# cbrl/BNN-PYNQ

Measured on AMD Instinct MI355X. Metric: images/sec (whole node) CNV-W1A1 CIFAR-10-shape batch, higher is better.
Workload: dtype u1; 1 GPU; cnvW1A1, 131072 synthetic 32x32x3 uint8 images per GPU per step, inputs resident in HBM, params cifar10/cnvW1A1; parallelism=dp1 (batch shards, no data-path collective)

## Files before the change

bnn-pynq_amd/bnn/abi.py:

```python
import ctypes as C
import os

ROOT = os.path.dirname(os.path.realpath(__file__))
PLATFORM = os.environ.get("BNN_PLATFORM", "mi355x")
LIB_DIR = os.environ.get("BNN_MI355X_LIBDIR") or os.path.join(ROOT, "libraries", PLATFORM)
PARAM_ROOT = os.path.join(ROOT, "params")

LEGACY = ["load_parameters", "inference", "inference_multiple", "inference_multiple_with_faults",
          "free_results", "deinit"]
EXT = ["bnn_mi355x_network", "bnn_mi355x_image_bytes", "bnn_mi355x_last_error", "bnn_mi355x_set_device",
       "bnn_mi355x_pack_params", "bnn_mi355x_export_params", "bnn_mi355x_import_params",
       "bnn_mi355x_inference_buffer", "bnn_mi355x_inference_raw", "bnn_mi355x_inference_device",
       "bnn_mi355x_reserve", "bnn_mi355x_set_fault_seed", "bnn_mi355x_last_faults", "bnn_mi355x_plan_faults",
       "bnn_mi355x_pack_params_faulty", "bnn_mi355x_debug_stage_output", "bnn_mi355x_profile",
       "bnn_mi355x_profile_read", "bnn_mi355x_stage_name", "bnn_mi355x_thumbnail_size", "bnn_mi355x_images_to_cifar",
       "bnn_mi355x_params_bytes", "bnn_mi355x_import_params_device", "bnn_mi355x_params_crc", "bnn_mi355x_chunk_plan",
       "bnn_mi355x_binarize_pack", "bnn_mi355x_fault_campaigns", "bnn_mi355x_last_campaign_faults",
       "bnn_mi355x_enumerate_faults", "bnn_mi355x_fault_sweep", "bnn_mi355x_last_sweep_stages",
       "bnn_mi355x_enumerate_act_faults", "bnn_mi355x_act_fault_sweep", "bnn_mi355x_last_act_sweep_stages",
       "bnn_mi355x_matrix_stages", "bnn_mi355x_act_noise_campaigns", "bnn_mi355x_last_act_noise_counts",
       "bnn_mi355x_last_act_noise_seeds", "bnn_mi355x_act_noise_mask", "bnn_mi355x_enumerate_input_faults",
       "bnn_mi355x_input_fault_sweep", "bnn_mi355x_last_input_sweep_stages", "bnn_mi355x_input_noise_campaigns",
       "bnn_mi355x_last_input_noise_counts", "bnn_mi355x_last_input_noise_seeds", "bnn_mi355x_input_noise_mask",
       "bnn_mi355x_sweep_profile", "bnn_mi355x_last_sweep_profile", "bnn_mi355x_mem_noise_campaigns",
       "bnn_mi355x_last_mem_noise_counts", "bnn_mi355x_last_mem_noise_seeds", "bnn_mi355x_mem_noise_mask",
       "bnn_mi355x_mem_noise_params", "bnn_mi355x_hardening_scheme", "bnn_mi355x_hardening_layout", "bnn_mi355x_hardened_site",
       "bnn_mi355x_hardened_mem_noise_mask", "bnn_mi355x_pack_params_hardened", "bnn_mi355x_hardened_mem_noise_campaigns",
       "bnn_mi355x_hardened_mem_noise_params", "bnn_mi355x_last_hardened_mem_noise_counts",
       "bnn_mi355x_last_hardened_mem_noise_seeds", "bnn_mi355x_exposure_mask", "bnn_mi355x_exposure_campaigns",
       "bnn_mi355x_exposure_params", "bnn_mi355x_last_exposure_counts", "bnn_mi355x_last_exposure_seeds", "bnn_mi355x_ecc_encode",
       "bnn_mi355x_ecc_decode", "bnn_mi355x_ecc_layout", "bnn_mi355x_ecc_check_site", "bnn_mi355x_ecc_exposure_mask",
       "bnn_mi355x_pack_params_ecc", "bnn_mi355x_ecc_exposure_campaigns", "bnn_mi355x_ecc_exposure_params",
       "bnn_mi355x_last_ecc_exposure_counts", "bnn_mi355x_last_ecc_exposure_seeds", "bnn_mi355x_ecc_repair",
       "bnn_mi355x_pack_params_repair", "bnn_mi355x_repair_exposure_campaigns", "bnn_mi355x_repair_exposure_params",
       "bnn_mi355x_last_repair_exposure_counts", "bnn_mi355x_last_repair_exposure_seeds", "bnn_mi355x_wecc_encode",
       "bnn_mi355x_wecc_decode", "bnn_mi355x_wecc_repair", "bnn_mi355x_wecc_layout", "bnn_mi355x_wecc_exposure_mask",
       "bnn_mi355x_pack_params_wecc", "bnn_mi355x_wecc_exposure_campaigns", "bnn_mi355x_wecc_exposure_params",
       "bnn_mi355x_last_wecc_exposure_counts", "bnn_mi355x_last_wecc_exposure_seeds", "bnn_mi355x_iwecc_layout",
       "bnn_mi355x_iwecc_site", "bnn_mi355x_pack_params_iwecc", "bnn_mi355x_iwecc_exposure_campaigns",
       "bnn_mi355x_iwecc_exposure_params", "bnn_mi355x_last_iwecc_exposure_counts", "bnn_mi355x_last_iwecc_exposure_seeds",
       "bnn_mi355x_tile_boxes", "bnn_mi355x_windows_to_cifar", "bnn_mi355x_classify_windows"]


def lib_path(network, runtime="python_sw", lib_dir=None):
    return os.path.join(lib_dir or LIB_DIR, "%s-%s-%s.so" % (runtime, network, PLATFORM))


def declare_legacy(L):
    ip, fp = C.POINTER(C.c_int), C.POINTER(C.c_float)
    L.load_parameters.argtypes = [C.c_char_p]
    L.load_parameters.restype = None
    L.inference.argtypes = [C.c_char_p, ip, C.c_int, fp]
    L.inference.restype = C.c_int
    L.inference_multiple.argtypes = [C.c_char_p, C.c_int, ip, fp, C.c_int]
    L.inference_multiple.restype = ip
    L.inference_multiple_with_faults.argtypes = [C.c_char_p, C.c_int, ip, fp, C.c_uint, C.c_int, C.c_int, ip, C.c_uint]
    L.inference_multiple_with_faults.restype = ip
    L.free_results.argtypes = [ip]
    L.free_results.restype = None
    L.deinit.argtypes = []
    L.deinit.restype = None


def declare_extensions(L):
# ... 212 lines not shown
```

bnn-pynq_amd/csrc/kernels.h:

```cpp
#pragma once
#include <hip/hip_runtime.h>
#include <stdint.h>

#include "topology.h"

namespace bnn {

struct CnvLaunch {
  const uint8_t *images;
  int n;
  void *buf0, *buf1;
  const uint32_t *rows[9];
  const uint8_t *l0_mfma;
  const uint8_t *l1_mfma;
  const uint8_t *conv_mfma;
  bool l1_literal;
  bool has_two;
  int16_t *scores;
  int32_t *classes;
  int number_class;
  hipStream_t stream;
  hipEvent_t *events;
  int last_stage;
  hipEvent_t t0, t1;
  unsigned *done_flag;
  unsigned done_seq;
};

struct LfcLaunch {
  const uint8_t *images;
  bool packed;
  int n;
  void *buf0, *buf1;
  const uint32_t *rows[4];
  uint64_t *words;
  int32_t *classes;
  int number_class;
  hipStream_t stream;
  hipEvent_t *events;
  int last_stage;
  hipEvent_t t0, t1;
  bool t_dispatch;
  unsigned *done_flag;
  unsigned done_seq;
};

constexpr int kL0TileOffset = 2 * 64 * 32, kL0BigBytes = 2 * 32 * 2 * 16;

constexpr int kCnvStages = 9;
constexpr int kLfcStages = 6;
const char *stage_name(bool is_cnv, int stage);

size_t stage_output_bytes(bool is_cnv, int abits, int stage, int *in_buf1);
void cnv_workspace_bytes(int abits, size_t *buf0, size_t *buf1);
void lfc_workspace_bytes(int abits, size_t *buf0, size_t *buf1);

constexpr size_t kL1MfmaWeights = 9 * 2 * 64 * 16, kL1MfmaBytes = kL1MfmaWeights + 2 * 2 * 16 * 4;
void l1_mfma_table(const uint32_t *rows, uint8_t *dst);

constexpr size_t kConvMfmaL2Off = kL1MfmaBytes, kConvMfmaL3Off = kConvMfmaL2Off + 9 * 4 * 64 * 16 + 4 * 32 * 4,
                 kTailMfmaL4Off = kConvMfmaL3Off + 18 * 4 * 64 * 16 + 4 * 32 * 4;
constexpr size_t kTailMfmaL5Off = kTailMfmaL4Off + 18 * 8 * 64 * 16 + 8 * 32 * 4, kTailMfmaL6Off = kTailMfmaL5Off + 36 * 8 * 64 * 16 + 8 * 32 * 4,
                 kTailMfmaL7Off = kTailMfmaL6Off + 4 * 16 * 64 * 16 + 16 * 32 * 4, kConvMfmaBytes = kTailMfmaL7Off + 8 * 16 * 64 * 16 + 16 * 32 * 4;
hipError_t conv_mfma_table(const uint32_t *const rows[9], uint8_t *dst, hipStream_t s);

constexpr size_t kConvMfmaA2L2Off = 9 * 2 * 64 * 16 + 2 * 64 * 4, kConvMfmaA2L3Off = kConvMfmaA2L2Off + 9 * 4 * 64 * 16 + 4 * 64 * 4,
                 kTailMfmaA2L4Off = kConvMfmaA2L3Off + 18 * 4 * 64 * 16 + 4 * 64 * 4;
constexpr size_t kTailMfmaA2L5Off = kTailMfmaA2L4Off + 18 * 8 * 64 * 16 + 8 * 64 * 4, kTailMfmaA2L6Off = kTailMfmaA2L5Off + 36 * 8 * 64 * 16 + 8 * 64 * 4,
                 kTailMfmaA2L7Off = kTailMfmaA2L6Off + 4 * 16 * 64 * 16 + 16 * 64 * 4, kConvMfmaA2Bytes = kTailMfmaA2L7Off + 8 * 16 * 64 * 16 + 16 * 64 * 4;
hipError_t conv_mfma_a2_table(NetId net, const uint32_t *const rows[9], uint8_t *dst, hipStream_t s);

int cnv_matrix_stages(NetId net, const CnvLaunch &a);

hipError_t run_cnv(NetId net, const CnvLaunch &a);
hipError_t run_lfc(NetId net, const LfcLaunch &a);

struct MultiSeg { int run, image, slot, len; };
struct MultiLaunch {
  const uint8_t *images;
  const MultiSeg *segs;
  int nsegs, max_len, total;
  int n;
  void *buf0, *buf1;
  const uint32_t *rows[9];
  const uint8_t *l0_mfma;
  size_t stride;
  bool has_two;
  int32_t *classes;
  uint64_t *words;
  int number_class;
  hipStream_t stream;
  int first = 0, last = 1 << 30;
};
hipError_t run_cnv_multi(NetId net, const MultiLaunch &a);
hipError_t run_lfc_multi(NetId net, const MultiLaunch &a);
// ... 65 lines not shown
```

bnn-pynq_amd/csrc/kernels.hip:

```cpp
#include <hip/hip_runtime.h>
#include <hip/hip_ext.h>
#include <stdint.h>

#include <cstdlib>
#include <cstring>
#include <type_traits>

#define BNN_HD __host__ __device__
#include "act_faults.h"
#include "input_faults.h"
#include "kernels.h"
#include "mem_faults.h"
#include "mem_org.h"
#include "packed_params.h"
static_assert(bnn::kL0TileOffset == (int)bnn::kL0MfmaTileOffset && bnn::kL0BigBytes == (int)bnn::kL0MfmaBigBytes,
              "k_conv0_tile's operand offsets must be the ones packed_params.cpp writes the layer-0 table by");

namespace bnn {
namespace {

typedef const uint32_t __attribute__((address_space(4))) *kptr32;
typedef const uint64_t __attribute__((address_space(4))) *kptr64;

constexpr int kBlock = 256;
// ... 595 lines not shown
        if (valid && h == 0 && !(c & 1)) gout[(size_t)(t0 >> 1) * NT + (c >> 1) * NT + mt] = ~pooled;
      } else {
        uint32_t nf[2];
#pragma unroll
        for (int dy = 0; dy < 2; dy++) {
          int v[16];
#pragma unroll
          for (int k = 0; k < 16; k++) v[k] = __float_as_int(acc[dy][k]);
          nf[dy] = sign_nibbles(v, h);
        }
        const auto sw = __builtin_amdgcn_permlane32_swap(nf[0], nf[1], false, false);
        if (valid) *reinterpret_cast<uint32_t *>(reinterpret_cast<char *>(gout) + ob) = ~(sw[0] | sw[1]);
      }
      x += DX, rp += DR, ps += 2 * DR * WS + DX;
      if constexpr (!POOL) ob += (2 * DR * WOUT + DX) * NT * 4;
      if (x >= WOUT) {
        x -= WOUT, rp += 1, ps += 2 * WS - WOUT;
        if constexpr (!POOL) ob += WOUT * NT * 4;
      }
      if (rp >= RP) rp -= RP, ps += IMGS - 2 * RP * WS;
    }
  }
}

__global__ __launch_bounds__(256) void k_conv_mfma_table(const uint32_t *__restrict__ rows, int row_dw, int ksteps, int tiles,
                                                          int mw, uint8_t *__restrict__ dst) {
  const int idx = blockIdx.x * 256 + threadIdx.x, nw = ksteps * tiles * 64;
  if (idx < nw) {
    const int ks = idx / (tiles * 64), mt = (idx / 64) % tiles, lane = idx & 63, n = 32 * mt + (lane & 31), h = lane >> 5;
    const uint32_t bits = rows[(size_t)n * row_dw + 2 + 2 * ks + h];
    reinterpret_cast<uint4 *>(dst)[idx] = make_uint4(fp4_pm1(bits & 255), fp4_pm1((bits >> 8) & 255), fp4_pm1((bits >> 16) & 255),
                                                     fp4_pm1(bits >> 24));
  } else if (idx < nw + tiles * 32) {
    const int j = idx - nw, mt = j >> 5, h = (j >> 4) & 1, reg = j & 15;
    const int n = 32 * mt + (reg & 3) + 8 * (reg >> 2) + 4 * h;
    long long t = (int)rows[(size_t)n * row_dw];
    t = t < -1 ? -1 : (t > mw + 2 ? mw + 2 : t);
    reinterpret_cast<float *>(dst + (size_t)nw * 16)[j] = (float)(-(mw - 2 * t) - 1);
  }
}

__device__ __forceinline__ uint32_t nibble_spread(uint32_t byte) {
  uint32_t t = byte & 0xFFu;
  t = (t | (t << 12)) & 0x000F000Fu;
  t = (t | (t << 6)) & 0x03030303u;
  return (t | (t << 3)) & 0x11111111u;
// ... 2044 lines not shown
  else return a.n >= conv_mfma_a2_min<ARITH>() ? a.conv_mfma : nullptr;
}
constexpr long long kTailMfmaMinW1A1 = 3072, kTailMfmaMinW1A2 = 3072, kTailMfmaMinW2A2 = 1024;
constexpr int kTailMfmaStages = 0xF0;
template <int ARITH>
inline long long tail_mfma_min() {
  static const long long v = [] {
    const char *e = std::getenv("BNN_MI355X_TAIL_MFMA_MIN");
    return e ? std::atoll(e) : (ARITH == AR_XNOR ? kTailMfmaMinW1A1 : ARITH == AR_TB ? kTailMfmaMinW1A2 : kTailMfmaMinW2A2);
  }();
  return v;
}
template <int ARITH>
inline const uint8_t *tail_mfma_for(const CnvLaunch &a) {
  if (a.done_flag && a.n == 1) return nullptr;
  return a.n >= tail_mfma_min<ARITH>() ? a.conv_mfma : nullptr;
}
inline unsigned persistent_grid(long long units, long long cap) {
  const long long per = (units + cap - 1) / cap;
  return (unsigned)((units + per - 1) / per);
}
constexpr long long kConvMfmaGrid = 512;
constexpr int kConvMfmaImgsL1 = 2, kConvMfmaImgs = 8;
constexpr int kTailMfmaImgsL4 = 32, kTailMfmaImgsL5 = 32, kTailMfmaImgsFc = 128;
constexpr long long kTailMfmaGrid8 = 256;
#define BNN_TAIL_MFMA(A2, KS, NT, CONV, WAVES, G, cap, in, out, tab)                                                               \
  hipLaunchKernelGGL((k_tail_mfma<A2, KS, NT, CONV, WAVES, G>), dim3(persistent_grid((n + (G) - 1) / (G), (cap))), dim3(64 * (WAVES)), 0, s, \
                     in, out, tab, (int)n)

inline int gpb_for(long long items, int groups) { return (items + kBlock - 1) / kBlock >= 2048 ? groups : 1; }

inline bool narrow_for(long long items, int groups32, long long limit) { return ((items + kBlock - 1) / kBlock) * groups32 < limit; }
constexpr long long kNarrowLimitCnv = 8192, kNarrowLimitLfc = 512;
constexpr long long kFcLastWaveMax = 32768;
constexpr long long kPixelLaneMax = 512;
constexpr long long kCnvTailMax = 1024;

inline dim3 grid_for(long long items, int groups) {
  const long long item_blocks = (items + kBlock - 1) / kBlock;
  return dim3((unsigned)(((item_blocks + 7) / 8) * 8 * groups));
}

#define BNN_LAUNCH(kern, grid, stream, ...)                                   \
  do {                                                                        \
    if ((grid).x > 0) hipLaunchKernelGGL(kern, grid, dim3(kBlock), 0, stream, __VA_ARGS__); \
  } while (0)
// ... 18 lines not shown
  if (a.l0_mfma) {
    const dim3 g0((unsigned)((n * 900 + kBlock - 1) / kBlock));
    if (a.last_stage >= 0) {
      if (n >= l0_tile_min()) BNN_LAUNCH((k_conv0_tile<OUT2>), dim3((unsigned)((n + kL0Imgs - 1) / kL0Imgs)), s, a.images, A, a.l0_mfma, (int)n);
      else BNN_LAUNCH((k_conv0_mfma<OUT2>), g0, s, a.images, A, a.l0_mfma, (int)(n * 900));
    }
  } else {
    if (a.last_stage >= 0) BNN_LAUNCH((k_conv0<OUT2>), grid_for(n * 900, 2 / gpb_for(n * 900, 2)), s, a.images, A, a.rows[0], (int)(n * 900), 2, gpb_for(n * 900, 2));
  }
  BNN_MARK(a.events, 1, s);
  if constexpr (ARITH == AR_XNOR && !OUT2) {
    const bool pix = n <= kPixelLaneMax;
    const uint8_t *const cm = conv_mfma_for<ARITH, OUT2>(a);
    const dim3 g1(persistent_grid((n + kConvMfmaImgsL1 - 1) / kConvMfmaImgsL1, kConvMfmaGrid)),
        gm(persistent_grid((n + kConvMfmaImgs - 1) / kConvMfmaImgs, kConvMfmaGrid));
    if (a.last_stage >= 1) {
      if (a.l1_literal) {
        BNN_LAUNCH(k_l1_literal, dim3((unsigned)((n * 784 + kBlock - 1) / kBlock)), s, A64, reinterpret_cast<uint64_t *>(B), a.rows[1], (int)(n * 784));
      } else if (a.l1_mfma) {
        const long long pairs = (n + 1) / 2;
        hipLaunchKernelGGL(k_l1_mfma, dim3((unsigned)(pairs < 512 ? pairs : 512)), dim3(256), 0, s, reinterpret_cast<const uint32_t *>(a.buf0), B,
                           a.l1_mfma, (int)n);
      } else if (cm) {
        hipLaunchKernelGGL((k_conv_mfma<30, 2, 2, true, kConvMfmaImgsL1>), g1, dim3(256), 0, s, reinterpret_cast<const uint32_t *>(a.buf0), B, cm,
                           (int)n);
      } else if (pix) BNN_LAUNCH((k_vec_x<9, true, 1, 30, 8, true>), grid_for(n * 784, 8), s, A64, B, a.rows[1], (int)(n * 784), 8, 1);
      else BNN_STAGE((k_quad_x<1, 30, true>), (k_quad_x<1, 30, true, 8>), n * 196, 2, A64, B, a.rows[1]);
    }
    BNN_MARK(a.events, 2, s);
    if (a.last_stage >= 2) {
      if (cm) hipLaunchKernelGGL((k_conv_mfma<14, 2, 4, false, kConvMfmaImgs>), gm, dim3(256), 0, s, B, A, cm + kConvMfmaL2Off, (int)n);
      else if (pix) BNN_LAUNCH((k_vec_x<9, true, 1, 14, 8>), grid_for(n * 144, 16), s, B64, A, a.rows[2], (int)(n * 144), 16, 1);
      else BNN_STAGE((k_quad_x<1, 14, false>), (k_quad_x<1, 14, false, 8>), n * 36, 4, B64, A, a.rows[2]);
    }
    BNN_MARK(a.events, 3, s);
    if (a.last_stage >= 3) {
      if (cm) hipLaunchKernelGGL((k_conv_mfma<12, 4, 4, true, kConvMfmaImgs>), gm, dim3(256), 0, s, A, B, cm + kConvMfmaL3Off, (int)n);
      else if (pix) BNN_LAUNCH((k_vec_x<18, true, 2, 12, 8, true>), grid_for(n * 100, 16), s, A64, B, a.rows[3], (int)(n * 100), 16, 1);
      else BNN_STAGE((k_quad_x<2, 12, true>), (k_quad_x<2, 12, true, 8>), n * 25, 4, A64, B, a.rows[3]);
    }
    BNN_MARK(a.events, 4, s);
    const uint8_t *const tm = tail_mfma_for<ARITH>(a);
    const uint32_t *const A32 = A, *const B32 = B;
    if (!tm && n <= kCnvTailMax && !a.events && a.last_stage >= kCnvStages - 1) {
      hipLaunchKernelGGL(k_cnv_tail, dim3((unsigned)n), dim3(512), 0, s, B64, a.scores, a.classes, a.rows[4], a.rows[5], a.rows[6],
                         a.rows[7], a.rows[8], a.number_class, n == 1 ? a.done_flag : nullptr, a.done_seq);
      return;
    }
    if (a.last_stage >= 4) {
      if (tm && (kTailMfmaStages & 16)) BNN_TAIL_MFMA(false, 18, 8, true, 8, kTailMfmaImgsL4, kTailMfmaGrid8, B32, A, tm + kTailMfmaL4Off);
      else BNN_STAGE((k_vec_x<18, true, 2, 5>), (k_vec_x<18, true, 2, 5, 8>), n * 9, 8, B64, A, a.rows[4]);
    }
    BNN_MARK(a.events, 5, s);
    if (a.last_stage >= 5) {
      if (tm && (kTailMfmaStages & 32)) BNN_TAIL_MFMA(false, 36, 8, false, 8, kTailMfmaImgsL5, kTailMfmaGrid8, A32, B, tm + kTailMfmaL5Off);
      else BNN_STAGE((k_vec_x<36, false, 1, 1>), (k_vec_x<36, false, 1, 1, 8>), n, 8, A64, B, a.rows[5]);
    }
    BNN_MARK(a.events, 6, s);
    if (a.last_stage >= 6) {
      if (tm && (kTailMfmaStages & 64)) BNN_TAIL_MFMA(false, 4, 16, false, 4, kTailMfmaImgsFc, kConvMfmaGrid, B32, A, tm + kTailMfmaL6Off);
// ... 208 lines not shown
                       p.tiles, 64 * p.ksteps, dst + p.off);
  }
  return hipGetLastError();
}

hipError_t conv_mfma_a2_table(NetId net, const uint32_t *const rows[9], uint8_t *dst, hipStream_t s) {
  const struct { int layer, ksteps, tiles; size_t off; } part[7] = {{1, 9, 2, 0},  {2, 9, 4, kConvMfmaA2L2Off},  {3, 18, 4, kConvMfmaA2L3Off}, {4, 18, 8, kTailMfmaA2L4Off},
                                                                   {5, 36, 8, kTailMfmaA2L5Off}, {6, 4, 16, kTailMfmaA2L6Off}, {7, 8, 16, kTailMfmaA2L7Off}};
  for (const auto &p : part) {
    const dim3 grid((unsigned)((p.ksteps * p.tiles * 64 + p.tiles * 64 + 255) / 256));
    if (net == NET_CNVW2A2) hipLaunchKernelGGL(k_conv_mfma_a2_table<true>, grid, dim3(256), 0, s, rows[p.layer], p.ksteps, p.tiles, dst + p.off);
    else hipLaunchKernelGGL(k_conv_mfma_a2_table<false>, grid, dim3(256), 0, s, rows[p.layer], p.ksteps, p.tiles, dst + p.off);
  }
  return hipGetLastError();
}

int cnv_matrix_stages(NetId net, const CnvLaunch &a) {
  switch (net) {
    case NET_CNVW1A1: return matrix_stages_t<AR_XNOR, false>(a);
    case NET_CNVW1A2: return matrix_stages_t<AR_TB, true>(a);
    case NET_CNVW2A2: return matrix_stages_t<AR_TT, true>(a);
    default: return 0;
  }
}

hipError_t run_cnv(NetId net, const CnvLaunch &a) {
  if (a.n <= 0) return hipSuccess;
  const bool marked = a.done_flag && a.n == 1;
  if (a.t0 && !marked) (void)hipEventRecord(a.t0, a.stream);
  switch (net) {
    case NET_CNVW1A1: run_cnv_t<AR_XNOR, false>(a); break;
    case NET_CNVW1A2: run_cnv_t<AR_TB, true>(a); break;
    case NET_CNVW2A2:
      if (a.has_two) run_cnv_t<AR_TT, true, true>(a);
      else run_cnv_t<AR_TT, true>(a);
      break;
    default: return hipErrorInvalidValue;
  }
  if (a.t1 && !marked) (void)hipEventRecord(a.t1, a.stream);
  return hipGetLastError();
}

hipError_t run_lfc(NetId net, const LfcLaunch &a) {
  if (a.n <= 0) return hipSuccess;
  const long long n = a.n, narrow_limit = kNarrowLimitLfc;
  uint32_t *A = reinterpret_cast<uint32_t *>(a.buf0), *B = reinterpret_cast<uint32_t *>(a.buf1);
// ... 315 lines not shown
```

bnn-pynq_amd/csrc/runtime.hip:

```cpp
#include <hip/hip_runtime.h>

#include <fcntl.h>
#if defined(__x86_64__)
#include <immintrin.h>
#endif
#include <sys/stat.h>
#include <sys/uio.h>
#include <sched.h>
#include <unistd.h>

#include <algorithm>
#include <atomic>
#include <chrono>
#include <condition_variable>
#include <mutex>
#include <cmath>
#include <cstdio>
#include <cstdlib>
#include <cstring>
#include <map>
#include <new>
#include <random>
#include <memory>
#include <string>
// ... 91 lines not shown
int largest_chunk(const std::vector<int> &base) {
  int m = 0;
  for (size_t c = 0; c + 1 < base.size(); c++) m = base[c + 1] - base[c] > m ? base[c + 1] - base[c] : m;
  return m;
}

struct Runtime {
  const NetSpec &spec = net_spec(BNN_NETWORK);
  int device = -1;
  std::string err;
  RawParams raw;
  std::vector<uint8_t> blob;
  void *d_blob = nullptr;
  size_t d_blob_bytes = 0;
  uint64_t fault_seed = 0;
  int debug_last_stage = -1;
  std::vector<Fault> last_faults;
  const uint32_t *rows[9] = {};
  const uint8_t *l0_mfma = nullptr;
  uint8_t *d_l1_mfma = nullptr;
  bool l1_mfma = false, l1_literal = false;
  uint8_t *d_conv_mfma = nullptr;
  bool conv_mfma = false, conv_xnor = false;
  bool warmed = false;
  int two_rows = 0;
  int cap = 0;
  void *buf0 = nullptr, *buf1 = nullptr;
  int cap2 = 0;
  void *buf0b = nullptr, *buf1b = nullptr;
  hipStream_t stream2 = nullptr;
  hipEvent_t lane2_done = nullptr;
  hipStream_t feed_aux = nullptr;
  int stage_cap = 0;
  int stage_slots = 0;
  uint8_t *d_images[kStageSlots] = {};
  size_t res_cap = 0;
  int16_t *d_scores = nullptr;
  int32_t *d_classes = nullptr;
  uint64_t *d_words = nullptr;
  hipStream_t stream = nullptr, copy_stream = nullptr;
  uint8_t *h_io = nullptr, *d_io = nullptr;
  hipEvent_t io_t0 = nullptr, io_t1 = nullptr;
  unsigned io_seq = 0;
  std::vector<uint8_t> h_scratch;
  int32_t *h_classes = nullptr;
  uint64_t *h_words = nullptr;
// ... 166 lines not shown
    HIP_OK(hipMalloc(&r.d_blob, r.blob.size()));
    r.d_blob_bytes = r.blob.size();
  }
  HIP_OK(hipDeviceSynchronize());
  HIP_OK(hipMemcpy(r.d_blob, r.blob.data(), r.blob.size(), hipMemcpyHostToDevice));
  r.two_rows = count_two_rows(r.spec, r.blob);
  const PackedHeader *h = reinterpret_cast<const PackedHeader *>(r.blob.data());
  for (int l = 0; l < r.spec.nlayers; l++)
    r.rows[l] = reinterpret_cast<const uint32_t *>(static_cast<const uint8_t *>(r.d_blob) + h->layer[l].offset);
  const char *l0 = std::getenv("BNN_MI355X_L0");
  const bool valu = l0 && std::strcmp(l0, "valu") == 0;
  r.l0_mfma = (h->l0_mfma_offset && !valu) ? static_cast<const uint8_t *>(r.d_blob) + h->l0_mfma_offset : nullptr;
  const char *l1 = std::getenv("BNN_MI355X_L1");
  r.l1_mfma = r.spec.id == NET_CNVW1A1 && l1 && std::strcmp(l1, "mfma") == 0;
  r.l1_literal = r.spec.id == NET_CNVW1A1 && l1 && std::strcmp(l1, "lds") == 0;
  if (r.l1_mfma) {
    std::vector<uint8_t> tab(kL1MfmaBytes);
    l1_mfma_table(reinterpret_cast<const uint32_t *>(r.blob.data() + h->layer[1].offset), tab.data());
    if (!r.d_l1_mfma) HIP_OK(hipMalloc(reinterpret_cast<void **>(&r.d_l1_mfma), kL1MfmaBytes));
    HIP_OK(hipMemcpy(r.d_l1_mfma, tab.data(), kL1MfmaBytes, hipMemcpyHostToDevice));
  }
  const char *cv = std::getenv("BNN_MI355X_CONV");
  r.conv_mfma = r.spec.is_cnv && !(cv && std::strcmp(cv, "valu") == 0);
  return make_conv_tables(r.stream);
}

void free_workspace() {
  Runtime &r = rt();
  if (r.cap == 0 && r.cap2 == 0 && r.stage_cap == 0 && r.res_cap == 0 && !r.d_pp_src && !r.d_pp_rec && !r.win_scene_cap && !r.win_meta_cap && !r.win_body_cap && !r.file_cap && !r.all_cap && !r.h_io &&
      !r.h_classes && !r.h_words && !r.copies_cap && !r.camp_cap && !r.camp_res_cap && !r.sw_base_cap && !r.sw_stage_cap &&
      !r.sw_segs_cap && !r.sw_alive_cap && !r.sw_res_cap && !r.sw_cnt_cap && !r.sw_diffs_cap && !r.sw_prof_cap && !r.noise_cap && !r.in_stage_cap)
    return;
  if (r.device >= 0) (void)hipSetDevice(r.device);
  (void)hipDeviceSynchronize();
  if (r.h_io) (void)hipHostFree(r.h_io);
  r.h_io = r.d_io = nullptr;
  if (r.h_classes) (void)hipHostFree(r.h_classes);
  if (r.h_words) (void)hipHostFree(r.h_words);
  r.h_classes = nullptr; r.h_words = nullptr;
  r.h_classes_cap = r.h_words_cap = 0;
  r.h_scratch = std::vector<uint8_t>();
  (void)hipFree(r.buf0); (void)hipFree(r.buf1);
  for (auto &b : r.d_images) { (void)hipFree(b); b = nullptr; }
  (void)hipFree(r.d_scores); (void)hipFree(r.d_classes); (void)hipFree(r.d_words);
  r.buf0 = r.buf1 = nullptr;
  r.d_scores = nullptr; r.d_classes = nullptr; r.d_words = nullptr;
// ... 222 lines not shown
    if (cap != hipStreamCaptureStatusNone) {
      hipStreamCaptureMode mode = hipStreamCaptureModeRelaxed;
      HIP_OK(hipThreadExchangeStreamCaptureMode(&mode));
      const hipError_t we = hipEventSynchronize(r.ws_event);
      (void)hipThreadExchangeStreamCaptureMode(&mode);
      if (we != hipSuccess)
        return fail("inference_device: an earlier call on another stream still owns the workspace and cannot be waited for during "
                    "stream capture; synchronise that stream before capturing");
    } else {
      HIP_OK(hipStreamWaitEvent(s, r.ws_event, 0));
    }
  }
  if (own >= 0) r.ws_seen[own] = r.ws_gen;
  else r.ws_pending = false;
  return 0;
}

void set_forms(CnvLaunch &a) {
  Runtime &r = rt();
  a.l0_mfma = r.l0_mfma;
  a.l1_mfma = r.l1_mfma ? r.d_l1_mfma : nullptr;
  a.l1_literal = r.l1_literal;
  a.conv_mfma = r.conv_mfma && !r.conv_xnor ? r.d_conv_mfma : nullptr;
  a.has_two = r.two_rows > 0;
}

int enqueue(const uint8_t *d_imgs, int n, int ncls, int32_t *d_classes, int16_t *d_scores, uint64_t *d_words,
            hipStream_t s, hipEvent_t t0 = nullptr, hipEvent_t t1 = nullptr, int lane = 0, bool t_dispatch = false, bool packed = false,
            unsigned *done_flag = nullptr, unsigned done_seq = 0) {
  Runtime &r = rt();
  hipError_t e;
  hipEvent_t *evs = nullptr;
  void *const ws0 = lane ? r.buf0b : r.buf0, *const ws1 = lane ? r.buf1b : r.buf1;
  if (n > (lane ? r.cap2 : r.cap)) return fail("internal: a chunk of " + std::to_string(n) + " images exceeds the activation workspace");
  if (settle_handover(s)) return -1;
  if (r.profiling) {
    const int need = (r.spec.is_cnv ? kCnvStages : kLfcStages) + 1;
    if (r.prof_used == r.prof_sets.size()) {
      std::vector<hipEvent_t> set(need);
      for (auto &ev : set) HIP_OK(hipEventCreate(&ev));
      r.prof_sets.push_back(set);
    }
    evs = r.prof_sets[r.prof_used++].data();
  }
  if (r.spec.is_cnv) {
    CnvLaunch a{};
// ... 845 lines not shown
    result = new (std::nothrow) int[(size_t)(n > 0 ? n : 1)];
    if (!result) { fail("out of memory"); return nullptr; }
    for (int i = 0; i < n; i++) result[i] = lfc_class_batched(w[i], ncls);
  }
  return result;
}

int *classify_host(const uint8_t *imgs, int n, int ncls, float *usec, int enable_detail) {
  return classify_with([&](int32_t *c, int16_t *s, uint64_t *w, const uint64_t **v) { return infer_host(imgs, n, ncls, c, s, w, usec, v); }, n, ncls,
                       enable_detail);
}

template <class T>
int copy_out(const std::vector<T> &v, T *out, int cap) {
  for (int i = 0; out && i < cap && i < (int)v.size(); i++) out[i] = v[(size_t)i];
  return (int)v.size();
}

}
}

#ifdef BNN_LFC_STAMPS
namespace bnn { hipError_t lfc_stamps_read(unsigned long long *dst); hipError_t lfc_wstamps_read(unsigned long long *dst); }
#endif
using namespace bnn;

extern "C" {

void load_parameters(const char *path) {
  Runtime &r = rt();
  std::printf("Setting network weights and thresholds in accelerator...\n");
  RawParams raw;
  const std::string e = read_raw_params(r.spec, path ? path : "", raw);
  if (!e.empty()) { fail(e); return; }
  r.raw = std::move(raw);
  pack_blob(r.spec, r.raw, r.blob);
  if (upload_blob()) { r.blob.clear(); return; }
  r.err.clear();
  (void)warm_up();
}

int inference(const char *path, int results[64], int number_class, float *usecPerImage) {
  Runtime &r = rt();
  if (!ready()) return -1;
  ImageFile f;
  trace().start();
// ... 2574 lines not shown
}

#ifdef BNN_LFC_STAMPS
int bnn_mi355x_debug_lfc_stamps(unsigned long long *dst) {
  if (hipDeviceSynchronize() != hipSuccess) return -1;
  return bnn::lfc_stamps_read(dst) == hipSuccess ? 0 : -1;
}
int bnn_mi355x_debug_lfc_wstamps(unsigned long long *dst) {
  if (hipDeviceSynchronize() != hipSuccess) return -1;
  return bnn::lfc_wstamps_read(dst) == hipSuccess ? 0 : -1;
}
#endif

int bnn_mi355x_matrix_stages(int n_images) {
  Runtime &r = rt();
  if (!r.d_blob) return -1;
  if (!r.spec.is_cnv || n_images <= 0) return 0;
  CnvLaunch a{};
  a.n = n_images;
  set_forms(a);
  return cnv_matrix_stages(r.spec.id, a);
}

int bnn_mi355x_chunk_plan(int n_images, int from_file, int *bases, int cap) {
  if (n_images < 0) return fail("chunk_plan: bad arguments");
  const std::vector<int> plan = plan_chunks(n_images, false, from_file != 0);
  for (size_t i = 0; i < plan.size() && (int)i < cap && bases; i++) bases[i] = plan[i];
  return (int)plan.size();
}

long bnn_mi355x_debug_stage_output(const uint8_t *images, int n_images, int stage, void *dst, size_t cap) {
  Runtime &r = rt();
  if (!ready()) return -1;
  int in_buf1 = 0;
  const size_t per = stage_output_bytes(r.spec.is_cnv, r.spec.abits, stage, &in_buf1);
  if (per == 0 || n_images <= 0 || n_images > kHostChunk || !images || !dst || cap < per * (size_t)n_images)
    return fail("debug_stage_output: bad arguments");
  r.debug_last_stage = stage;
  std::vector<uint64_t> w((size_t)n_images);
  const int rc = infer_host(images, n_images, 10, nullptr, nullptr, r.spec.is_cnv ? nullptr : w.data(), nullptr);
  r.debug_last_stage = -1;
  if (rc) return -1;
  HIP_OK(hipMemcpy(dst, in_buf1 ? r.buf1 : r.buf0, per * (size_t)n_images, hipMemcpyDeviceToHost));
  return (long)per;
}

// ... 350 lines not shown
```

include/bnn_mi355x.h:

```cpp
#ifndef BNN_MI355X_H
#define BNN_MI355X_H

#include <stddef.h>
#include <stdint.h>

#ifdef __cplusplus
extern "C" {
#endif


void load_parameters(const char *path);

int inference(const char *path, int results[64], int number_class, float *usecPerImage);

int *inference_multiple(const char *path, int number_class, int *image_number, float *usecPerImage,
                        int enable_detail);

int *inference_multiple_with_faults(const char *path, int number_class, int *image_number,
                                    float *usecPerImage, unsigned int flip_count, int word_size,
                                    int target, int *target_layers, unsigned int num_targets);

void free_results(int *result);

void deinit(void);
// ... 8 lines not shown

size_t bnn_mi355x_pack_params(const char *path, void *dst, size_t cap);
size_t bnn_mi355x_export_params(void *dst, size_t cap);
int bnn_mi355x_import_params(const void *src, size_t bytes);
size_t bnn_mi355x_params_bytes(void);
int bnn_mi355x_import_params_device(const void *d_src, size_t bytes, void *hip_stream);
unsigned int bnn_mi355x_params_crc(void);

int *bnn_mi355x_inference_buffer(const uint8_t *images, int n_images, int number_class,
                                 float *usecPerImage, int enable_detail);

int bnn_mi355x_binarize_pack(const uint8_t *images, int n_images, uint64_t *words);

int bnn_mi355x_inference_raw(const uint8_t *images, int n_images, int16_t *scores, uint64_t *words,
                             float *usecPerImage);

int bnn_mi355x_inference_device(const void *d_images, int n_images, int number_class, int32_t *d_classes,
                                int16_t *d_scores, uint64_t *d_words, void *hip_stream);
int bnn_mi355x_reserve(int max_images);

int bnn_mi355x_chunk_plan(int n_images, int from_file, int *bases, int cap);

int bnn_mi355x_matrix_stages(int n_images);

int bnn_mi355x_set_fault_seed(unsigned long long seed);
int bnn_mi355x_last_faults(int *records, int cap_records);
int *bnn_mi355x_fault_campaigns(const char *path, int number_class, int num_runs, unsigned long long seed,
                                unsigned int flip_count, int word_size, int target, const int *target_layers,
                                unsigned int num_targets, int *image_number, float *usecPerImage);
int bnn_mi355x_last_campaign_faults(int *records, int cap_records);
int bnn_mi355x_plan_faults(unsigned long long seed, int num_images, unsigned int flip_count, int word_size, int target,
                           const int *target_layers, unsigned int num_targets, int *records, int cap_records);
size_t bnn_mi355x_pack_params_faulty(const char *path, const int *records, int n_faults, void *dst, size_t cap);
long bnn_mi355x_enumerate_faults(int layer, int target, int word_size, long first, int *records, int cap_records);
long bnn_mi355x_fault_sweep(const char *path, int number_class, const int *records, int n_faults, int *changed, int *diffs,
                            long cap_diffs, int *image_number, float *usecPerImage);
int bnn_mi355x_last_sweep_stages(long *pairs_per_stage, int cap);
long bnn_mi355x_enumerate_act_faults(int layer, long first, int *records, int cap_records);
long bnn_mi355x_act_fault_sweep(const char *path, int number_class, const int *records, int n_faults, int *changed, int *diffs,
                                long cap_diffs, int *image_number, float *usecPerImage);
int bnn_mi355x_last_act_sweep_stages(long *pairs_per_stage, int cap);

int *bnn_mi355x_act_noise_campaigns(const char *path, int number_class, int num_runs, unsigned long long seed,
                                    const unsigned int *rate_q32, int n_rates, int *image_number, float *usecPerImage);
int bnn_mi355x_last_act_noise_counts(long *upsets, int cap);
int bnn_mi355x_last_act_noise_seeds(unsigned long long *seeds, int cap);
// ... 143 lines not shown
```

Measured before the change: 40.81 million images/s.

## Add software-pipelined rotated-tile MFMA conv kernel for first conv layer

Result: no change. 40.74 million images/s (median of 3 runs) (-0.2%).

```diff
diff --git a/bnn-pynq_amd/bnn/abi.py b/bnn-pynq_amd/bnn/abi.py
--- a/bnn-pynq_amd/bnn/abi.py
+++ b/bnn-pynq_amd/bnn/abi.py
@@ -39,7 +39,8 @@
        "bnn_mi355x_last_wecc_exposure_counts", "bnn_mi355x_last_wecc_exposure_seeds", "bnn_mi355x_iwecc_layout",
        "bnn_mi355x_iwecc_site", "bnn_mi355x_pack_params_iwecc", "bnn_mi355x_iwecc_exposure_campaigns",
        "bnn_mi355x_iwecc_exposure_params", "bnn_mi355x_last_iwecc_exposure_counts", "bnn_mi355x_last_iwecc_exposure_seeds",
-       "bnn_mi355x_tile_boxes", "bnn_mi355x_windows_to_cifar", "bnn_mi355x_classify_windows"]
+       "bnn_mi355x_tile_boxes", "bnn_mi355x_windows_to_cifar", "bnn_mi355x_classify_windows",
+       "bnn_mi355x_rotated_tile_stages"]
 
 
 def lib_path(network, runtime="python_sw", lib_dir=None):
diff --git a/bnn-pynq_amd/csrc/kernels.h b/bnn-pynq_amd/csrc/kernels.h
--- a/bnn-pynq_amd/csrc/kernels.h
+++ b/bnn-pynq_amd/csrc/kernels.h
@@ -25,6 +25,7 @@
   hipEvent_t t0, t1;
   unsigned *done_flag;
   unsigned done_seq;
+  int conv_tile;
 };
 
 struct LfcLaunch {
@@ -71,6 +72,7 @@
 hipError_t conv_mfma_a2_table(NetId net, const uint32_t *const rows[9], uint8_t *dst, hipStream_t s);
 
 int cnv_matrix_stages(NetId net, const CnvLaunch &a);
+int cnv_rotated_tile_stages(NetId net, const CnvLaunch &a);
 
 hipError_t run_cnv(NetId net, const CnvLaunch &a);
 hipError_t run_lfc(NetId net, const LfcLaunch &a);
diff --git a/bnn-pynq_amd/csrc/kernels.hip b/bnn-pynq_amd/csrc/kernels.hip
--- a/bnn-pynq_amd/csrc/kernels.hip
+++ b/bnn-pynq_amd/csrc/kernels.hip
@@ -641,6 +641,218 @@
     }
   }
 }
+
+#ifdef BNN_CONV_STAMPS
+constexpr int kConvStampGroups = 4, kConvStampTiles = 16, kConvStampGroupWords = 2 + 3 * kConvStampTiles;
+constexpr int kConvStampWords = 2 + kConvStampGroups * kConvStampGroupWords;
+__device__ __forceinline__ unsigned long long conv_stamp() {
+  unsigned long long t;
+  __builtin_amdgcn_sched_barrier(0);
+  asm volatile("s_memtime %0\n\ts_waitcnt lgkmcnt(0)" : "=s"(t)::"memory");
+  __builtin_amdgcn_sched_barrier(0);
+  return t;
+}
+#define CONV_STAMP_ARG , unsigned long long *__restrict__ stamps
+#else
+#define CONV_STAMP_ARG
+#endif
+#ifndef BNN_CONV_P_PRIO
+#define BNN_CONV_P_PRIO 0
+#endif
+
+template <int WIN, int CD, int NT, bool POOL, int G>
+__global__ __launch_bounds__(256, 2) void k_conv_mfma_p(const uint32_t *__restrict__ in, uint32_t *__restrict__ out,
+                                                         const uint8_t *__restrict__ tab, int n_images CONV_STAMP_ARG) {
+  constexpr int WOUT = WIN - 2, RP = WOUT / 2, IPI = RP * WOUT, KH = CD / 2, KS = 9 * KH, NS = 3 * KH, STREAMS = 4 / NT;
+  constexpr int PIX = WIN * WIN, DWI = PIX * CD, NPF = (G * DWI + 255) / 256;
+  constexpr int WS = conv_mfma_row_stride(WIN), PIXS = WIN * WS, IMGS = conv_mfma_img_stride(WIN, CD);
+  static_assert(WOUT % 2 == 0 && IPI % 2 == 0 && (NT == 2 || NT == 4), "tile geometry");
+  __shared__ uint4 plane[G * IMGS];
+  __shared__ uint32_t lut[256];
+  const int tid = threadIdx.x, lane = tid & 63, wave = __builtin_amdgcn_readfirstlane(tid >> 6), mt = wave % NT, c = lane & 31, h = lane >> 5;
+  lut[tid] = fp4_pm1((uint32_t)tid);
+  const uint4 *__restrict__ wt = reinterpret_cast<const uint4 *>(tab);
+  v8i wreg[KS];
+#pragma unroll
+  for (int ks = 0; ks < KS; ks++) {
+    const uint4 v = wt[(ks * NT + mt) * 64 + lane];
+    wreg[ks] = v8i{(int)v.x, (int)v.y, (int)v.z, (int)v.w, 0, 0, 0, 0};
+  }
+  const v16f seed = reinterpret_cast<const v16f *>(tab + (size_t)KS * NT * 64 * 16)[mt * 2 + h];
+  const int ngroups = (n_images + G - 1) / G;
+  uint32_t pre[NPF];
+  auto fetch = [&](int grp) {
+    const int img0 = grp * G, lim = min(G, n_images - img0) * DWI;
+#pragma unroll
+    for (int j = 0; j < NPF; j++) {
+      const int d = tid + 256 * j;
+      pre[j] = d < lim ? in[(size_t)img0 * DWI + d] : 0u;
+    }
+  };
+  auto slot = [&](int d) {
+    const int i = d / DWI, e = d - i * DWI, pix = e / CD, q = e % CD;
+    return i * IMGS + q * PIXS + (WS == WIN ? pix : pix / WIN * WS + pix % WIN);
+  };
+  constexpr int STEP = 32 * STREAMS, DR = STEP / WOUT, DX = STEP % WOUT, PS_LAST = (G - 1) * IMGS + 2 * (RP - 1) * WS + WOUT - 1;
+  static_assert(DX % 2 == 0 && DR + 1 <= RP, "a lane's column keeps its parity; one row-pair wrap and one image wrap per step");
+  const int item0 = (wave / NT) * 32 + c, i0 = item0 / IPI, rem0 = item0 - i0 * IPI, rp0 = rem0 / WOUT, x0 = rem0 - rp0 * WOUT;
+  const int ps0 = i0 * IMGS + 2 * rp0 * WS + x0;
+  const uint32_t ob0 = (uint32_t)((i0 * (WOUT * WOUT) + (2 * rp0 + h) * WOUT + x0) * NT + mt) * 4;
+#if BNN_CONV_P_PRIO == 3
+  const bool odd_slot = __builtin_amdgcn_s_getreg((3 << 11) | 4) & 1;
+  if (odd_slot) __builtin_amdgcn_s_setprio(2);
+#endif
+#ifdef BNN_CONV_STAMPS
+  unsigned long long *__restrict__ const st = stamps + (size_t)(blockIdx.x * 4 + wave) * kConvStampWords;
+  if (stamps && lane == 0) {
+    st[0] = __builtin_amdgcn_s_getreg((31 << 11) | 4);
+    st[1] = __builtin_amdgcn_s_getreg((31 << 11) | 20);
+  }
+  int sgi = 0;
+#endif
+  if (blockIdx.x < ngroups) fetch(blockIdx.x);
+  for (int grp = blockIdx.x; grp < ngroups; grp += gridDim.x) {
+    const int img0 = grp * G, nimg = min(G, n_images - img0), nitems = nimg * IPI;
+    uint32_t *__restrict__ gout = out + (size_t)img0 * (POOL ? RP * RP : WOUT * WOUT) * NT;
+#ifdef BNN_CONV_STAMPS
+    const bool sg = stamps && sgi < kConvStampGroups;
+    unsigned long long *__restrict__ const sp = st + 2 + sgi * kConvStampGroupWords;
+    int sti = 0;
+    const unsigned long long sb0 = conv_stamp();
+#endif
+    __syncthreads();
+#pragma unroll
+    for (int j = 0; j < NPF; j++) {
+      const int d = tid + 256 * j;
+      if (d < nimg * DWI) {
+        const uint32_t bits = pre[j];
+        plane[slot(d)] = make_uint4(lut[bits & 255], lut[(bits >> 8) & 255], lut[(bits >> 16) & 255], lut[bits >> 24]);
+      }
+    }
+    if (grp + (int)gridDim.x < ngroups) fetch(grp + gridDim.x);
+    __syncthreads();
+#ifdef BNN_CONV_STAMPS
+    const unsigned long long sb1 = conv_stamp();
+    if (sg && lane == 0) sp[0] = sb0, sp[1] = sb1;
+#endif
+    int x = x0, rp = rp0, ps = ps0;
+    [[maybe_unused]] uint32_t ob = ob0;
+    int t0 = (wave / NT) * 32;
+    if (t0 < nitems) {
+      auto tile_planes = [&](int slot0) {
+        uint32_t pb = (uint32_t)min(slot0, PS_LAST) * 16 + (uint32_t)h * (PIXS * 16);
+        asm("" : "+v"(pb));
+        return reinterpret_cast<const uint4 *>(reinterpret_cast<const char *>(plane) + pb);
+      };
+      const uint4 *__restrict__ P = tile_planes(ps);
+      auto read = [&](v8i &b, int s, int y) {
+        const uint4 v = P[(s / 3) * 2 * PIXS + y * WS + s % 3];
+        b = v8i{(int)v.x, (int)v.y, (int)v.z, (int)v.w, 0, 0, 0, 0};
+      };
+      v8i b[2][4];
+#pragma unroll
+      for (int y = 0; y < 4; y++) read(b[0][y], 0, y);
+      do {
+        v16f acc[2] = {seed, seed};
+        auto mfma = [&](const v8i (&bb)[4], int s, int k) {
+          acc[k & 1] = __builtin_amdgcn_mfma_scale_f32_32x32x64_f8f6f4(wreg[((k >> 1) * 3 + s % 3) * KH + s / 3], bb[(k >> 1) + (k & 1)], acc[k & 1], 4,
+                                                                      4, 0, 0x7F7F7F7F, 0, 0x7F7F7F7F);
+        };
+#ifdef BNN_CONV_STAMPS
+        const unsigned long long s0 = conv_stamp();
+#endif
+#if BNN_CONV_P_PRIO == 1
+        __builtin_amdgcn_s_setprio(1);
+#elif BNN_CONV_P_PRIO == 2
+        __builtin_amdgcn_s_setprio(0);
+#endif
+#pragma unroll
+        for (int s = 0; s < NS; s++)
+#pragma unroll
+          for (int k = 0; k < 6; k++) {
+            __builtin_amdgcn_sched_barrier(0);
+            mfma(b[s & 1], s, k);
+            if (s + 1 < NS && k < 4) read(b[(s + 1) & 1][k], s + 1, k);
+          }
+        __builtin_amdgcn_sched_barrier(0);
+#if BNN_CONV_P_PRIO == 1
+        __builtin_amdgcn_s_setprio(0);
+#elif BNN_CONV_P_PRIO == 2
+        __builtin_amdgcn_s_setprio(1);
+#endif
+#ifdef BNN_CONV_STAMPS
+        const unsigned long long s1 = conv_stamp();
+#endif
+        const bool valid = c < nitems - t0;
+        [[maybe_unused]] const uint32_t ob_t = ob;
+        const int tp = t0;
+        const bool wx = x >= WOUT - DX;
+        x += wx ? DX - WOUT : DX, rp += wx ? DR + 1 : DR, ps += wx ? 2 * (DR + 1) * WS + DX - WOUT : 2 * DR * WS + DX;
+        if constexpr (!POOL) ob += (wx ? 2 * DR * WOUT + DX + WOUT : 2 * DR * WOUT + DX) * NT * 4;
+        const bool wr = rp >= RP;
+        rp -= wr ? RP : 0, ps += wr ? IMGS - 2 * RP * WS : 0;
+        P = tile_planes(ps);
+#pragma unroll
+        for (int y = 0; y < 4; y++) read(b[0][y], 0, y);
+        __builtin_amdgcn_sched_barrier(0);
+        if constexpr (POOL) {
+          int v[16];
+#pragma unroll
+          for (int k = 0; k < 16; k++) v[k] = __float_as_int(acc[0][k]) & __float_as_int(acc[1][k]);
+          const uint32_t nf = or_halves(sign_nibbles(v, h));
+          const uint32_t pooled = nf & (uint32_t)__builtin_amdgcn_mov_dpp((int)nf, 0xB1, 0xF, 0xF, true);
+          if (valid && h == 0 && !(c & 1)) gout[(size_t)(tp >> 1) * NT + (c >> 1) * NT + mt] = ~pooled;
+        } else {
+          uint32_t nf[2];
+#pragma unroll
+          for (int dy = 0; dy < 2; dy++) {
+            int v[16];
+#pragma unroll
+            for (int k = 0; k < 16; k++) v[k] = __float_as_int(acc[dy][k]);
+            nf[dy] = sign_nibbles(v, h);
+          }
+          const auto sw = __builtin_amdgcn_permlane32_swap(nf[0], nf[1], false, false);
+          if (valid) *reinterpret_cast<uint32_t *>(reinterpret_cast<char *>(gout) + ob_t) = ~(sw[0] | sw[1]);
+        }
+#ifdef BNN_CONV_STAMPS
+        const unsigned long long s2 = conv_stamp();
+        if (sg && sti < kConvStampTiles && lane == 0) sp[2 + 3 * sti] = s0, sp[3 + 3 * sti] = s1, sp[4 + 3 * sti] = s2;
+        sti++;
+#endif
+        t0 += STEP;
+      } while (t0 < nitems);
+    }
+#ifdef BNN_CONV_STAMPS
+    sgi++;
+#endif
+  }
+}
+
+#ifdef BNN_CONV_STAMPS
+}
+static unsigned long long *g_conv_stamps[3];
+static size_t g_conv_stamp_words[3], g_conv_stamp_cap[3];
+unsigned long long *conv_stamps_for(int layer, unsigned blocks, hipStream_t s) {
+  const size_t words = (size_t)blocks * 4 * kConvStampWords;
+  if (words > g_conv_stamp_cap[layer]) {
+    (void)hipFree(g_conv_stamps[layer]);
+    if (hipMalloc(reinterpret_cast<void **>(&g_conv_stamps[layer]), words * 8) != hipSuccess) return g_conv_stamps[layer] = nullptr, nullptr;
+    g_conv_stamp_cap[layer] = words;
+  }
+  g_conv_stamp_words[layer] = words;
+  (void)hipMemsetAsync(g_conv_stamps[layer], 0, words * 8, s);
+  return g_conv_stamps[layer];
+}
+long long conv_stamps_read(int layer, unsigned long long *dst, long long cap_words) {
+  if (layer < 0 || layer > 2 || !g_conv_stamps[layer] || (long long)g_conv_stamp_words[layer] > cap_words) return -1;
+  if (hipMemcpy(dst, g_conv_stamps[layer], g_conv_stamp_words[layer] * 8, hipMemcpyDeviceToHost) != hipSuccess) return -1;
+  return (long long)g_conv_stamp_words[layer] / kConvStampWords;
+}
+namespace {
+#define CONV_STAMPS_FOR(layer, grid) , conv_stamps_for(layer, (grid).x, s)
+#else
+#define CONV_STAMPS_FOR(layer, grid)
+#endif
 
 __global__ __launch_bounds__(256) void k_conv_mfma_table(const uint32_t *__restrict__ rows, int row_dw, int ksteps, int tiles,
                                                           int mw, uint8_t *__restrict__ dst) {
@@ -2731,6 +2943,14 @@
 }
 constexpr long long kConvMfmaGrid = 512;
 constexpr int kConvMfmaImgsL1 = 2, kConvMfmaImgs = 8;
+constexpr bool kConvTileP[3] = {true, false, false};
+inline bool conv_tile_p(const CnvLaunch &a, int l) { return a.conv_tile == 2 || (a.conv_tile == 0 && kConvTileP[l]); }
+#define BNN_CONV_MFMA(L, WIN, CD, NT, POOL, G, grid, in, out, tab)                                                                     \
+  do {                                                                                                                             \
+    if (conv_tile_p(a, L))                                                                                                         \
+      hipLaunchKernelGGL((k_conv_mfma_p<WIN, CD, NT, POOL, G>), grid, dim3(256), 0, s, in, out, tab, (int)n CONV_STAMPS_FOR(L, grid)); \
+    else hipLaunchKernelGGL((k_conv_mfma<WIN, CD, NT, POOL, G>), grid, dim3(256), 0, s, in, out, tab, (int)n);                    \
+  } while (0)
 constexpr int kTailMfmaImgsL4 = 32, kTailMfmaImgsL5 = 32, kTailMfmaImgsFc = 128;
 constexpr long long kTailMfmaGrid8 = 256;
 #define BNN_TAIL_MFMA(A2, KS, NT, CONV, WAVES, G, cap, in, out, tab)                                                               \
@@ -2795,20 +3015,19 @@
         hipLaunchKernelGGL(k_l1_mfma, dim3((unsigned)(pairs < 512 ? pairs : 512)), dim3(256), 0, s, reinterpret_cast<const uint32_t *>(a.buf0), B,
                            a.l1_mfma, (int)n);
       } else if (cm) {
-        hipLaunchKernelGGL((k_conv_mfma<30, 2, 2, true, kConvMfmaImgsL1>), g1, dim3(256), 0, s, reinterpret_cast<const uint32_t *>(a.buf0), B, cm,
-                           (int)n);
+        BNN_CONV_MFMA(0, 30, 2, 2, true, kConvMfmaImgsL1, g1, reinterpret_cast<const uint32_t *>(a.buf0), B, cm);
       } else if (pix) BNN_LAUNCH((k_vec_x<9, true, 1, 30, 8, true>), grid_for(n * 784, 8), s, A64, B, a.rows[1], (int)(n * 784), 8, 1);
       else BNN_STAGE((k_quad_x<1, 30, true>), (k_quad_x<1, 30, true, 8>), n * 196, 2, A64, B, a.rows[1]);
     }
     BNN_MARK(a.events, 2, s);
     if (a.last_stage >= 2) {
-      if (cm) hipLaunchKernelGGL((k_conv_mfma<14, 2, 4, false, kConvMfmaImgs>), gm, dim3(256), 0, s, B, A, cm + kConvMfmaL2Off, (int)n);
+      if (cm) BNN_CONV_MFMA(1, 14, 2, 4, false, kConvMfmaImgs, gm, B, A, cm + kConvMfmaL2Off);
       else if (pix) BNN_LAUNCH((k_vec_x<9, true, 1, 14, 8>), grid_for(n * 144, 16), s, B64, A, a.rows[2], (int)(n * 144), 16, 1);
       else BNN_STAGE((k_quad_x<1, 14, false>), (k_quad_x<1, 14, false, 8>), n * 36, 4, B64, A, a.rows[2]);
     }
     BNN_MARK(a.events, 3, s);
     if (a.last_stage >= 3) {
-      if (cm) hipLaunchKernelGGL((k_conv_mfma<12, 4, 4, true, kConvMfmaImgs>), gm, dim3(256), 0, s, A, B, cm + kConvMfmaL3Off, (int)n);
+      if (cm) BNN_CONV_MFMA(2, 12, 4, 4, true, kConvMfmaImgs, gm, A, B, cm + kConvMfmaL3Off);
       else if (pix) BNN_LAUNCH((k_vec_x<18, true, 2, 12, 8, true>), grid_for(n * 100, 16), s, A64, B, a.rows[3], (int)(n * 100), 16, 1);
       else BNN_STAGE((k_quad_x<2, 12, true>), (k_quad_x<2, 12, true, 8>), n * 25, 4, A64, B, a.rows[3]);
     }
@@ -3063,6 +3282,11 @@
     case NET_CNVW2A2: return matrix_stages_t<AR_TT, true>(a);
     default: return 0;
   }
+}
+
+int cnv_rotated_tile_stages(NetId net, const CnvLaunch &a) {
+  if (net != NET_CNVW1A1 || !conv_mfma_for<AR_XNOR, false>(a)) return 0;
+  return (conv_tile_p(a, 0) && !a.l1_literal && !a.l1_mfma ? 2 : 0) | (conv_tile_p(a, 1) ? 4 : 0) | (conv_tile_p(a, 2) ? 8 : 0);
 }
 
 hipError_t run_cnv(NetId net, const CnvLaunch &a) {
diff --git a/bnn-pynq_amd/csrc/runtime.hip b/bnn-pynq_amd/csrc/runtime.hip
--- a/bnn-pynq_amd/csrc/runtime.hip
+++ b/bnn-pynq_amd/csrc/runtime.hip
@@ -137,6 +137,7 @@
   bool l1_mfma = false, l1_literal = false;
   uint8_t *d_conv_mfma = nullptr;
   bool conv_mfma = false, conv_xnor = false;
+  int conv_tile = 0;
   bool warmed = false;
   int two_rows = 0;
   int cap = 0;
@@ -349,6 +350,8 @@
   }
   const char *cv = std::getenv("BNN_MI355X_CONV");
   r.conv_mfma = r.spec.is_cnv && !(cv && std::strcmp(cv, "valu") == 0);
+  const char *ct = std::getenv("BNN_MI355X_CONV_TILE");
+  r.conv_tile = !ct ? 0 : std::strcmp(ct, "v1") == 0 ? 1 : std::strcmp(ct, "p") == 0 ? 2 : 0;
   return make_conv_tables(r.stream);
 }
 
@@ -617,6 +620,7 @@
   a.l1_mfma = r.l1_mfma ? r.d_l1_mfma : nullptr;
   a.l1_literal = r.l1_literal;
   a.conv_mfma = r.conv_mfma && !r.conv_xnor ? r.d_conv_mfma : nullptr;
+  a.conv_tile = r.conv_tile;
   a.has_two = r.two_rows > 0;
 }
 
@@ -1508,6 +1512,9 @@
 
 #ifdef BNN_LFC_STAMPS
 namespace bnn { hipError_t lfc_stamps_read(unsigned long long *dst); hipError_t lfc_wstamps_read(unsigned long long *dst); }
+#endif
+#ifdef BNN_CONV_STAMPS
+namespace bnn { long long conv_stamps_read(int layer, unsigned long long *dst, long long cap_words); }
 #endif
 using namespace bnn;
 
@@ -4128,6 +4135,23 @@
   return cnv_matrix_stages(r.spec.id, a);
 }
 
+int bnn_mi355x_rotated_tile_stages(int n_images) {
+  Runtime &r = rt();
+  if (!r.d_blob) return -1;
+  if (!r.spec.is_cnv || n_images <= 0) return 0;
+  CnvLaunch a{};
+  a.n = n_images;
+  set_forms(a);
+  return cnv_rotated_tile_stages(r.spec.id, a);
+}
+
+#ifdef BNN_CONV_STAMPS
+long long bnn_mi355x_debug_conv_stamps(int layer, unsigned long long *dst, long long cap_words) {
+  if (hipDeviceSynchronize() != hipSuccess) return -1;
+  return bnn::conv_stamps_read(layer, dst, cap_words);
+}
+#endif
+
 int bnn_mi355x_chunk_plan(int n_images, int from_file, int *bases, int cap) {
   if (n_images < 0) return fail("chunk_plan: bad arguments");
   const std::vector<int> plan = plan_chunks(n_images, false, from_file != 0);
diff --git a/include/bnn_mi355x.h b/include/bnn_mi355x.h
--- a/include/bnn_mi355x.h
+++ b/include/bnn_mi355x.h
@@ -54,6 +54,7 @@
 int bnn_mi355x_chunk_plan(int n_images, int from_file, int *bases, int cap);
 
 int bnn_mi355x_matrix_stages(int n_images);
+int bnn_mi355x_rotated_tile_stages(int n_images);
 
 int bnn_mi355x_set_fault_seed(unsigned long long seed);
 int bnn_mi355x_last_faults(int *records, int cap_records);
```
